# MingXiangL/SPE

Measured on AMD Instinct MI355X. Metric: images/sec (whole node) at 3x800x1333 bs=2/GPU, higher is better.
Workload: dtype bf16/fp16 operands, fp32 accumulate; 1 GPU; TSCAM_cait_S24 (C=384, depth 24, 8 heads) + 0-layer encoder + 6-layer conditional-DETR decoder x2 stages, 100 queries, COCO heads (91), 2x3x800x1333 per GPU (N=4150 tokens), fwd + SetCriterion + SetCriterionRefine + bwd + grad all-reduce + clip + AdamW; global_batch=2, parallelism=dp1

## Files before the change

### spe_amd/csrc/attn_flash_bwd.hip

```cpp
#include "attn_flash_common.h"

#define FLB_NW 4
#define FLB_HB 4
#define FLB_GWR 144
#define FLB_NK16 3
#define FLB_RSFUSE 1
#define FLB_DQAHEAD 2
#define FLB_SB_NOMEM 0x00F
#define FLB_PHASE() __builtin_amdgcn_sched_barrier(0)
#ifndef SPE_ABLATE
#undef FLB_DBG_SAMETILE
#undef FLB_DBG_NOST
#undef FLB_DBG_STAMP
#endif
#ifdef FLB_DBG_STAMP
#define FLB_STAMP(k) asm volatile("s_memtime %0\n\ts_waitcnt lgkmcnt(0)" : "=s"(stamp[k]))
#else
#define FLB_STAMP(k)
#endif
#ifndef FLB_STAGGER
#define FLB_STAGGER 1
#endif

struct FlashBwdArgs {
// ... 430 lines not shown
                for (int g = 0; g < H; ++g)
#pragma unroll
                    for (int dt = 0; dt < DT; ++dt) *reinterpret_cast<f32x4_t*>(dst + (g * DT + dt) * 256 + lane * 4) = dQ[g][dt];
            }
        }
        s += seg;
    }

#ifdef FLB_DBG_STAMP
    if (blockIdx.x == 0 && threadIdx.x == 0) {
        unsigned long long* o = reinterpret_cast<unsigned long long*>(a.dS);
        for (int k = 0; k < 5; ++k) o[k] = stacc[k];
        o[5] = stn;
    }
#endif
    {
        constexpr int NWG = 2 * (H * H + H);
        float* row = a.ws_w + ((long)blockIdx.x * NW + wave) * NWG;
        const f32x4_t dsum = (gwacc[0] + gwacc[1]) + (gwacc[2] + gwacc[3]);
        const int nn = lane & 15;
#pragma unroll
        for (int r = 0; r < 4; ++r) {
            const int g = 4 * (lane >> 4) + r;
            if (g < H && nn < H) row[g * H + nn] = FL_LN2 * dsum[r];
        }
#pragma unroll
        for (int g = 0; g < H; ++g) {
            const float v = spe_wave_sum(gb[g]);
            if (lane == 0) row[H * H + g] = v;
        }
    }
}

__global__ __launch_bounds__(256) void bwdq_dq_merge_kernel(const float* __restrict__ ws, float* __restrict__ O, unsigned short* __restrict__ O16,
                                                            long ob, long on, long oh, int B, int H, int N, int nt, int dh, int DT, int nmaj, int spw,
                                                            float scale, long nvec) {
    const long i = (long)blockIdx.x * 256 + threadIdx.x;
    if (i >= nvec) return;
    const int lane = (int)(i & 63);
    long r = i >> 6;
    const int dt = (int)(r % DT); r /= DT;
    const int g = (int)(r % H); r /= H;
    const int wave = (int)(r % FLB_NW); r /= FLB_NW;
    const long bm = r;
    const int b = (int)(bm / nmaj), mj = (int)(bm % nmaj);
    const int qt = mj * FLB_NW + wave;
    const int q = qt * 16 + (lane & 15), d = dt * 16 + 4 * (lane >> 4);
    if (qt >= nt || q >= N || d >= dh) return;
    const int first_wg = (int)((bm * nt) / spw), last_wg = (int)(((bm + 1) * nt - 1) / spw);
    const long slot_stride = (long)FLB_NW * H * DT * 256;
    const float* src = ws + bm * FL_MAXSLOT * slot_stride + ((long)wave * H + g) * (long)(DT * 256) + dt * 256 + lane * 4;
    f32x4_t acc = {0.f, 0.f, 0.f, 0.f};
    for (int sl = 0; sl <= last_wg - first_wg; ++sl) acc += *reinterpret_cast<const f32x4_t*>(src + sl * slot_stride);
    acc *= scale;
    const long oi = (long)b * ob + (long)q * on + (long)g * oh + d;
#pragma unroll
    for (int k = 0; k < 4; ++k) {
        if (d + k >= dh) break;
        if (O) O[oi + k] = acc[k];
    }
    if (O16) {
        if (d + 3 < dh && ((ob | on | oh) & 3) == 0 && ((reinterpret_cast<uintptr_t>(O16) & 7) == 0)) {
            const unsigned short h0 = spe_f2bf(acc[0]), h1 = spe_f2bf(acc[1]), h2 = spe_f2bf(acc[2]), h3 = spe_f2bf(acc[3]);
            *reinterpret_cast<uint2*>(O16 + oi) = make_uint2((unsigned)h0 | ((unsigned)h1 << 16), (unsigned)h2 | ((unsigned)h3 << 16));
        } else {
#pragma unroll
            for (int k = 0; k < 4; ++k) { if (d + k >= dh) break; O16[oi + k] = spe_f2bf(acc[k]); }
        }
    }
}

struct FlashBwdKArgs {
    const unsigned char* Qf; const unsigned char* dOf; const unsigned char* dO16;
    const unsigned char* Kf; const unsigned char* Vf;
    const float* Wl; const float* Ww; const float* bw;
    const float* c0; int Np;
    float* ws_d;
    float* ws_v;
    float* ws_w;
    const unsigned* keepbits;
    int B, N, nt, nmaj, spw; long total;
    float p_drop;
};

__device__ __forceinline__ void flb_rowsum4(const f32x4_t (&t)[4], f32x4_t& o) {
    float a0, a1, a2, a3, b0, b1, b2, b3;
    asm("s_nop 1\n\t"
        "v_add_f32_dpp %0, %12, %12 row_ror:8 row_mask:0xf bank_mask:0x3\n\t"
        "v_add_f32_dpp %1, %13, %13 row_ror:8 row_mask:0xf bank_mask:0x3\n\t"
        "v_add_f32_dpp %2, %14, %14 row_ror:8 row_mask:0xf bank_mask:0x3\n\t"
        "v_add_f32_dpp %3, %15, %15 row_ror:8 row_mask:0xf bank_mask:0x3\n\t"
        "v_add_f32_dpp %0, %20, %20 row_ror:8 row_mask:0xf bank_mask:0xc\n\t"
        "v_add_f32_dpp %1, %21, %21 row_ror:8 row_mask:0xf bank_mask:0xc\n\t"
        "v_add_f32_dpp %2, %22, %22 row_ror:8 row_mask:0xf bank_mask:0xc\n\t"
        "v_add_f32_dpp %3, %23, %23 row_ror:8 row_mask:0xf bank_mask:0xc\n\t"
        "v_add_f32_dpp %4, %16, %16 row_ror:8 row_mask:0xf bank_mask:0x3\n\t"
        "v_add_f32_dpp %5, %17, %17 row_ror:8 row_mask:0xf bank_mask:0x3\n\t"
        "v_add_f32_dpp %6, %18, %18 row_ror:8 row_mask:0xf bank_mask:0x3\n\t"
        "v_add_f32_dpp %7, %19, %19 row_ror:8 row_mask:0xf bank_mask:0x3\n\t"
        "v_add_f32_dpp %4, %24, %24 row_ror:8 row_mask:0xf bank_mask:0xc\n\t"
        "v_add_f32_dpp %5, %25, %25 row_ror:8 row_mask:0xf bank_mask:0xc\n\t"
        "v_add_f32_dpp %6, %26, %26 row_ror:8 row_mask:0xf bank_mask:0xc\n\t"
// ... 480 lines not shown
#pragma unroll
            for (int dt = 0; dt < DT; ++dt) flb_acc_fence(dV[g][dt]);
        if (wvalid) {
            float* dst = a.ws_v + (((long)bm * FL_MAXSLOT + slot) * NW + wave) * (long)(H * DT * 256);
#pragma unroll
            for (int g = 0; g < H; ++g)
#pragma unroll
                for (int dt = 0; dt < DT; ++dt) *reinterpret_cast<f32x4_t*>(dst + (g * DT + dt) * 256 + lane * 4) = dV[g][dt];
        }
        s += seg;
    }

#ifdef FLB_DBG_STAMP
    if (blockIdx.x == 0 && threadIdx.x == 0) {
        unsigned long long* o = reinterpret_cast<unsigned long long*>(a.ws_w);
        for (int k = 0; k < 6; ++k) o[k] = stacc[k];
        o[6] = stn;
    }
#endif
    {
        constexpr int NWG = 2 * (H * H + H);
        float* row = a.ws_w + ((long)blockIdx.x * NW + wave) * NWG + (H * H + H);
        const f32x4_t dsum = (gwacc[0] + gwacc[1]) + (gwacc[2] + gwacc[3]);
        const int nn = lane & 15;
#pragma unroll
        for (int r = 0; r < 4; ++r) {
            const int g = 4 * (lane >> 4) + r;
            if (g < H && nn < H) row[g * H + nn] = dsum[r] * (1.0f / FL_PD_SCALE);
            if (g < H && nn == H) row[H * H + g] = dsum[r];
        }
    }
}

__global__ __launch_bounds__(256) void bwdk_rows_merge_kernel(const float* __restrict__ ws, float* __restrict__ out, int B, int H, int N, int Np, int nmaj) {
    const long i = (long)blockIdx.x * 256 + threadIdx.x;
    const long per = (long)Np * H;
    if (i >= (long)B * per) return;
    const long bq = i / H; const int q = (int)(bq % Np), b = (int)(bq / Np);
    if (q >= N) { out[i] = 0.f; return; }
    const float* src = ws + (long)b * nmaj * per + (i - (long)b * per);
    float acc = 0.f;
    int m = 0;
    for (; m + 8 <= nmaj; m += 8) {
        float v[8];
#pragma unroll
        for (int k = 0; k < 8; ++k) v[k] = src[(long)(m + k) * per];
#pragma unroll
        for (int k = 0; k < 8; ++k) acc += v[k];
    }
    for (; m < nmaj; ++m) acc += src[(long)m * per];
    out[i] = acc;
}

constexpr int flbq_lds_bytes(int H, int DT, bool drop) {
    return (4 + FLB_NK16) * H * DT * 512 + 512 + FLB_NW * 3 * 4 * H * FLB_GWR + (drop ? 2048 : 0);
}
constexpr int flbk_lds_bytes(int H, int DT, bool drop) {
    return (4 + FLB_NK16) * H * DT * 512 + 2048 + 2 * FLB_NW * 16 * H * 4 + 512 + FLB_NW * 3 * 4 * H * FLB_GWR + (drop ? 2048 : 0);
}

static int dispatch_bwdq(const FlashBwdArgs& a, int H, int dh, int nwg, hipStream_t st) {
    return attn_dispatch(H, dh, [&](auto h, auto ds, auto tl) {
        constexpr int HH = decltype(h)::value, DS = decltype(ds)::value, DT = FragDims<DS, decltype(tl)::value>::DT;
        constexpr bool TL = decltype(tl)::value;
        if constexpr (flbq_lds_bytes(HH, DT, true) > FL_LDS_MAX) return -2;
        else return fl_launch<FlashBwdArgs, talking_bwdq_kernel<HH, DS, TL, true>, talking_bwdq_kernel<HH, DS, TL, false>>(
            a, nwg, 64 * FLB_NW, flbq_lds_bytes(HH, DT, false), flbq_lds_bytes(HH, DT, true), a.p_drop > 0.f, st);
    });
}

extern "C" int spe_talking_bwdq_plan(int B, int N, int nwg, int* steps_per_wg, int* nwg_used, int* nmajor) {
    const int nt = (N + 15) / 16;
    if ((long)B * nt <= 0 || nwg <= 0) { *steps_per_wg = 0; *nwg_used = 0; *nmajor = 0; return 0; }
    const FlashPlan p = fl_plan(B, nt, FLB_NW, nt, nwg);
    *steps_per_wg = p.spw; *nwg_used = p.nwg; *nmajor = p.nmaj;
    return 0;
}

static int bwdq_fill(FlashBwdArgs& a, FlashPlan& p, const void* Qf, const void* dOf, const void* Kf, const void* Vf, const void* K16, const float* Wl,
                     const float* Ww, const float* c0, int Np, const void* keepbits, int B, int H, int N, int dh, int nwg, float p_drop) {
    const int nt = (N + 15) / 16;
    if (dh < 1 || dh > 64 || nwg <= 0 || Np < nt * 16 || (p_drop > 0.f && !keepbits)) return -2;
    p = fl_plan(B, nt, FLB_NW, nt, nwg);
    a.Qf = (const unsigned char*)Qf; a.dOf = (const unsigned char*)dOf; a.Kf = (const unsigned char*)Kf; a.Vf = (const unsigned char*)Vf;
// ... 29 lines not shown
    return attn_dispatch(H, dh, [&](auto h, auto ds, auto tl) {
        constexpr int HH = decltype(h)::value, DS = decltype(ds)::value, DT = FragDims<DS, decltype(tl)::value>::DT;
        constexpr bool TL = decltype(tl)::value;
        if constexpr (flbk_lds_bytes(HH, DT, true) > FL_LDS_MAX) return -2;
        else return fl_launch<FlashBwdKArgs, talking_bwdk_kernel<HH, DS, TL, true>, talking_bwdk_kernel<HH, DS, TL, false>>(
            a, nwg, 64 * FLB_NW, flbk_lds_bytes(HH, DT, false), flbk_lds_bytes(HH, DT, true), a.p_drop > 0.f, st);
    });
}

extern "C" int spe_talking_fused_supported(int H, int dh) {
    return attn_dispatch(H, dh, [](auto h, auto ds, auto tl) {
        constexpr int HH = decltype(h)::value, DT = FragDims<decltype(ds)::value, decltype(tl)::value>::DT;
        return (flf_lds_bytes(HH, DT, true) <= FL_LDS_MAX && flbq_lds_bytes(HH, DT, true) <= FL_LDS_MAX && flbk_lds_bytes(HH, DT, true) <= FL_LDS_MAX) ? 0 : -2;
    }) == 0;
}

extern "C" int spe_talking_bwdk_pass1(const void* Qf, const void* dOf, const void* dO16, const void* Kf, const void* Vf, const float* Wl, const float* Ww,
                                      const float* bw, const float* c0, int Np, float* ws_d, float* ws_v, float* ws_w, float* Drows, float* dv, void* dv16,
                                      long ob, long on, long oh, const void* keepbits, int B, int H, int N, int dh, int nwg, float p_drop, hipStream_t st) {
    const int nt = (N + 15) / 16;
    if ((long)B * nt <= 0) return 0;
    if (dh < 1 || dh > 64 || nwg <= 0 || Np < nt * 16 + 64 || (p_drop > 0.f && !keepbits)) return -2;
    if (!Qf || !dOf || !dO16 || !Kf || !Vf || !Wl || !Ww || !bw || !c0 || !ws_d || !ws_v || !ws_w || !Drows || (!dv && !dv16)) return -2;
    const FlashPlan p = fl_plan(B, nt, FLB_NW, nt, nwg);
    FlashBwdKArgs a;
    a.Qf = (const unsigned char*)Qf; a.dOf = (const unsigned char*)dOf; a.dO16 = (const unsigned char*)dO16;
    a.Kf = (const unsigned char*)Kf; a.Vf = (const unsigned char*)Vf; a.Wl = Wl; a.Ww = Ww; a.bw = bw; a.c0 = c0; a.Np = Np;
    a.ws_d = ws_d; a.ws_v = ws_v; a.ws_w = ws_w;
    a.keepbits = (p_drop > 0.f) ? reinterpret_cast<const unsigned*>(keepbits) : nullptr;
    a.B = B; a.N = N; a.nt = nt; a.nmaj = p.nmaj; a.spw = p.spw; a.total = p.total; a.p_drop = p_drop;
    int rc = dispatch_bwdk(a, H, dh, p.nwg, st);
    if (rc != 0) return rc;
    const long n = (long)B * Np * H;
    hipLaunchKernelGGL(bwdk_rows_merge_kernel, dim3((unsigned)((n + 255) / 256)), dim3(256), 0, st, ws_d, Drows, B, H, N, Np, p.nmaj);
    SPE_CHECK_LAUNCH();
    const int DT = frag_geom(dh).dt;
    const long nvec = (long)B * p.nmaj * FLB_NW * H * DT * 64;
    hipLaunchKernelGGL(bwdq_dq_merge_kernel, dim3((unsigned)((nvec + 255) / 256)), dim3(256), 0, st, ws_v, dv, reinterpret_cast<unsigned short*>(dv16),
                       ob, on, oh, B, H, N, nt, dh, DT, p.nmaj, p.spw, 1.0f / FL_PD_SCALE, nvec);
    SPE_CHECK_LAUNCH();
    return 0;
}
```

### spe_amd/csrc/decoder_kv.hip

```cpp
#include <cstdlib>
#include "common.h"
#include "attn_pack.h"
#include "det_reduce.h"

typedef unsigned int kvu32x4_t __attribute__((ext_vector_type(4)));
typedef _Float16 kvh4_t __attribute__((ext_vector_type(4)));

__device__ __forceinline__ float kv_h2f(unsigned short h) { return (float)__builtin_bit_cast(_Float16, h); }

struct KvFragArgs {
    const unsigned short* ym; long ldm; const unsigned short* yp; long ldp;
    unsigned short* Kf; unsigned short* V16; unsigned short* K16; unsigned short* Vf;
    int L, B, S, H, dh, nt;
};

#define KV_MAXDH 64
__global__ __launch_bounds__(256) void kv_frag_kernel(KvFragArgs a) {
    __shared__ __attribute__((aligned(16))) unsigned short sK[4][16 * (2 * KV_MAXDH + 8)];
    __shared__ __attribute__((aligned(16))) unsigned short sV[4][16 * (KV_MAXDH + 8)];
    const int lane = threadIdx.x & 63, wave = __builtin_amdgcn_readfirstlane(threadIdx.x >> 6);
    const int dh = a.dh, dk = 2 * dh, d = a.H * dh, nt = a.nt, S = a.S;
    const int LDK = dk + 8, LDV = dh + 8;
    const int PPK = dk / 8, PPV = dh / 8, PPR = PPK + PPV;
    const int steps_k = (dk + 31) / 32, steps_v = (dh + 31) / 32, DTk = (dk + 15) / 16, DTv = (dh + 15) / 16;
// ... 96 lines not shown
extern "C" int spe_kv_grad_scatter(const float* dk, const float* dv, void* dYm, long ldm, void* dYp, long ldp, int layer, int B, int S,
                                   int H, int dh, hipStream_t st) {
    const long rows = (long)B * S;
    if (rows <= 0) return 0;
    if ((dh & 3) || (ldm & 3) || (ldp & 3) || layer < 0) return -2;
    const long n = rows * H * 3 * (dh / 4);
    long nb = (n + 255) / 256; if (nb > 8192) nb = 8192;
    hipLaunchKernelGGL(kv_grad_scatter_kernel, dim3((unsigned)nb), dim3(256), 0, st, dk, dv, reinterpret_cast<unsigned short*>(dYm), ldm,
                       reinterpret_cast<unsigned short*>(dYp), ldp, layer, rows, H, dh);
    SPE_CHECK_LAUNCH();
    return 0;
}


#define KV_MAXBLK 32
struct ColsumBlkArgs { const unsigned short* x; long ld; long R; int nblk, blkC, accumulate; float* out[KV_MAXBLK]; };
__global__ __launch_bounds__(256) void colsum_bf16_blocks_kernel(ColsumBlkArgs a, DetWs ws) {
    __shared__ float red[4][64];
    const int cl = threadIdx.x & 63, rl = threadIdx.x >> 6;
    const int C = a.nblk * a.blkC, c = blockIdx.x * 64 + cl;
    float acc = 0.f;
    if (c < C)
        for (long r = (long)blockIdx.y * 4 + rl; r < a.R; r += (long)gridDim.y * 4) acc += spe_bf2f(a.x[r * a.ld + c]);
    red[rl][cl] = acc;
    __syncthreads();
    det_reduce(ws, blockIdx.x, blockIdx.y, gridDim.y, 64, threadIdx.x, 256,
               [&](int k) { return red[0][k] + red[1][k] + red[2][k] + red[3][k]; },
               [&](int k, float s) {
                   const int cc = blockIdx.x * 64 + k;
                   if (cc < C) { float* o = a.out[cc / a.blkC] + cc % a.blkC; *o = a.accumulate ? *o + s : s; }
               });
}

__global__ __launch_bounds__(256) void colsum_bf16_blocks_v8_kernel(ColsumBlkArgs a, DetWs ws) {
    __shared__ float red[8][256 + 8];
    const int cg = threadIdx.x & 31, rl = threadIdx.x >> 5;
    const int C = a.nblk * a.blkC, c0 = blockIdx.x * 256 + cg * 8;
    float acc[8] = {0.f, 0.f, 0.f, 0.f, 0.f, 0.f, 0.f, 0.f};
    if (c0 < C) {
        const long rows_per = (a.R + gridDim.y - 1) / gridDim.y;
        const long r0 = (long)blockIdx.y * rows_per, r1 = r0 + rows_per < a.R ? r0 + rows_per : a.R;
        for (long r = r0 + rl; r < r1; r += 8) {
            const uint4 q = *reinterpret_cast<const uint4*>(a.x + r * a.ld + c0);
            const unsigned w[4] = {q.x, q.y, q.z, q.w};
#pragma unroll
            for (int i = 0; i < 4; ++i) { acc[2 * i] += __uint_as_float(w[i] << 16); acc[2 * i + 1] += __uint_as_float(w[i] & 0xffff0000u); }
        }
    }
#pragma unroll
    for (int i = 0; i < 8; ++i) red[rl][cg * 8 + i] = acc[i];
    __syncthreads();
    det_reduce(ws, blockIdx.x, blockIdx.y, gridDim.y, 256, threadIdx.x, 256,
               [&](int k) { float t = 0.f;
#pragma unroll
                            for (int j = 0; j < 8; ++j) t += red[j][k];
                            return t; },
               [&](int k, float s) {
                   const int cc = blockIdx.x * 256 + k;
                   if (cc < C) { float* o = a.out[cc / a.blkC] + cc % a.blkC; *o = a.accumulate ? *o + s : s; }
               });
}

extern "C" int spe_colsum_bf16_blocks(const void* x, long ld, long R, int nblk, int blkC, float* const* outs, int accumulate, hipStream_t st) {
    if (nblk <= 0 || blkC <= 0 || R <= 0) return 0;
    if (nblk > KV_MAXBLK) return -2;
    ColsumBlkArgs a;
    a.x = (const unsigned short*)x; a.ld = ld; a.R = R; a.nblk = nblk; a.blkC = blkC; a.accumulate = accumulate;
    for (int i = 0; i < nblk; ++i) a.out[i] = outs[i];
    if (((nblk * blkC) & 7) == 0 && (ld & 7) == 0 && (reinterpret_cast<uintptr_t>(x) & 15) == 0) {
        const int gx = (nblk * blkC + 255) / 256;
        static const int ry_max = SPE_KNOB("SPE_COLSUM_RY", 96);
        long ry = (R + 63) / 64; if (ry > ry_max) ry = ry_max; if (ry < 1) ry = 1;
        while (gx * ry > 1024 && ry > 16) ry /= 2;
        DetWs ws = spe_detws();
        DetDeferSeg sg[KV_MAXBLK];
        for (int i = 0; i < nblk; ++i) sg[i] = DetDeferSeg{outs[i], blkC};
        float* region = det_defer_try(gx, ry, 256, nblk, sg, st);
        if (region) ws.defer = region; else DET_CHECK(ws, gx, ry, 256);
        hipLaunchKernelGGL(colsum_bf16_blocks_v8_kernel, dim3(gx, (unsigned)ry), dim3(256), 0, st, a, ws);
        if (region) det_defer_commit(region, gx, ry, 256, nblk, sg, accumulate);
        SPE_CHECK_LAUNCH();
        return 0;
    }
    const int gx = (nblk * blkC + 63) / 64;
    long ry = (R + 255) / 256; if (ry > 64) ry = 64; if (ry < 1) ry = 1;
    const DetWs ws = spe_detws();
    DET_CHECK(ws, gx, ry, 64);
    hipLaunchKernelGGL(colsum_bf16_blocks_kernel, dim3(gx, (unsigned)ry), dim3(256), 0, st, a, ws);
    SPE_CHECK_LAUNCH();
    return 0;
}
```

### spe_amd/csrc/rowops.hip

```cpp
#include "common.h"
#include "det_reduce.h"

#define LN_MAXV 4

__device__ __forceinline__ void ln_store4(float4 v, float mu, float rs, float4 g, float4 b, long ro, int c, float* __restrict__ y,
                                          unsigned short* __restrict__ y16, unsigned short* __restrict__ y16lo, bool lo_f16) {
    float4 o;
    o.x = (v.x - mu) * rs * g.x + b.x; o.y = (v.y - mu) * rs * g.y + b.y;
    o.z = (v.z - mu) * rs * g.z + b.z; o.w = (v.w - mu) * rs * g.w + b.w;
    reinterpret_cast<float4*>(y + ro)[c] = o;
    if (y16) {
        const uint2 h = spe_pack_bf16x4(o);
        *reinterpret_cast<uint2*>(y16 + ro + 4 * c) = h;
        if (y16lo) {
            const float ov[4] = {o.x, o.y, o.z, o.w};
            *reinterpret_cast<uint2*>(y16lo + ro + 4 * c) = spe_second16(ov, h, lo_f16);
        }
    }
}

template <bool RES>
__global__ __launch_bounds__(256) void ln_fwd_kernel(const float* __restrict__ x, const float* __restrict__ z,
                                                     const float* __restrict__ gamma, const float* __restrict__ beta,
                                                     float* __restrict__ sum, float* __restrict__ y,
                                                     float* __restrict__ mean, float* __restrict__ rstd,
                                                     long R, int C, float eps, unsigned short* __restrict__ y16,
                                                     unsigned short* __restrict__ y16lo, bool lo_f16, float p, uint64_t seed, uint64_t offset) {
    const int lane = threadIdx.x & 63;
    const long row = (long)blockIdx.x * 4 + (threadIdx.x >> 6);
    if (row >= R) return;
    const int C4 = C >> 2;
    const float4* xr = reinterpret_cast<const float4*>(x + row * C);
    float4 v[LN_MAXV];
    float s = 0.f;
#pragma unroll
    for (int i = 0; i < LN_MAXV; ++i) {
// ... 35 lines not shown
    const int C4 = C >> 2, ldr = C + 4;
#pragma unroll
    for (int i = 0; i < MAXV; ++i) {
        const int c = lane + 64 * i;
        if (c < C4) {
#pragma unroll
            for (int k = 0; k < K; ++k) {
                float* r = red + (long)(k * NW + w) * ldr + 4 * c;
                r[0] = acc[k][i].x; r[1] = acc[k][i].y; r[2] = acc[k][i].z; r[3] = acc[k][i].w;
            }
        }
    }
    __syncthreads();
    auto set_of = [&](int c) {
        int k = 0;
#pragma unroll
        for (int j = 1; j < K; ++j) k += c >= j * C;
        return k;
    };
    det_reduce(ws, 0, blockIdx.x, gridDim.x, K * C, threadIdx.x, NW * 64,
               [&](int c) {
                   const int k = set_of(c), cc = c - k * C;
                   float t = 0.f;
#pragma unroll
                   for (int wv = 0; wv < NW; ++wv) t += red[(long)(k * NW + wv) * ldr + cc];
                   return t;
               },
               [&](int c, float t) {
                   const int k = set_of(c);
                   store(k, c - k * C, t);
               });
}

template <int NW, bool LS, int MAXV>
__global__ __launch_bounds__(NW * 64) void ln_bwd_kernel(const float* __restrict__ dy, const float* __restrict__ x,
                                                     const float* __restrict__ gamma, const float* __restrict__ mean,
                                                     const float* __restrict__ rstd, float* __restrict__ dx,
                                                     float* __restrict__ dgamma, float* __restrict__ dbeta,
                                                     long R, int C, const float* __restrict__ add, float* __restrict__ dz,
                                                     float p, uint64_t seed, uint64_t offset, DetWs ws, const float* __restrict__ dy2,
                                                     const float* __restrict__ ls_y, const float* __restrict__ ls_gamma,
                                                     unsigned short* __restrict__ ls_dy16, float* __restrict__ ls_db, float* __restrict__ ls_dg) {
    extern __shared__ float red_raw[];
    const int lane = threadIdx.x & 63, w = threadIdx.x >> 6;
    const int C4 = C >> 2;
    const float4* g4 = reinterpret_cast<const float4*>(gamma);
    float4 ag[MAXV], ab[MAXV];
    float4 lg[LS ? MAXV : 1], lb[LS ? MAXV : 1];
#pragma unroll
    for (int i = 0; i < MAXV; ++i) { ag[i] = make_float4(0, 0, 0, 0); ab[i] = make_float4(0, 0, 0, 0); }
#pragma unroll
    for (int i = 0; i < (LS ? MAXV : 1); ++i) { lg[i] = make_float4(0, 0, 0, 0); lb[i] = make_float4(0, 0, 0, 0); }
    for (long row = (long)blockIdx.x * NW + w; row < R; row += (long)gridDim.x * NW) {
        const float4* xr = reinterpret_cast<const float4*>(x + row * C);
        const float4* dr = reinterpret_cast<const float4*>(dy + row * C);
        const float4* dr2 = dy2 ? reinterpret_cast<const float4*>(dy2 + row * C) : nullptr;
        const float mu = mean[row], rs = rstd[row];
        float4 xh[MAXV], dg[MAXV];
        float s1 = 0.f, s2 = 0.f;
#pragma unroll
        for (int i = 0; i < MAXV; ++i) {
            const int c = lane + 64 * i;
            if (c < C4) {
                const float4 xv = xr[c], g = g4[c];
                float4 dv = dr[c];
                if (dr2) dv = spe_add4(dv, dr2[c]);
                xh[i].x = (xv.x - mu) * rs; xh[i].y = (xv.y - mu) * rs; xh[i].z = (xv.z - mu) * rs; xh[i].w = (xv.w - mu) * rs;
                dg[i] = spe_mul4(dv, g);
                s1 += spe_hsum(dg[i]);
                s2 += dg[i].x * xh[i].x + dg[i].y * xh[i].y + dg[i].z * xh[i].z + dg[i].w * xh[i].w;
                spe_fma4(ag[i], dv, xh[i]);
                ab[i] = spe_add4(ab[i], dv);
            }
        }
        s1 = spe_wave_sum(s1) / (float)C;
        s2 = spe_wave_sum(s2) / (float)C;
        float4* dxr = reinterpret_cast<float4*>(dx + row * C);
        const float4* ar = add ? reinterpret_cast<const float4*>(add + row * C) : nullptr;
#pragma unroll
        for (int i = 0; i < MAXV; ++i) {
            const int c = lane + 64 * i;
            if (c < C4) {
                float4 o;
                o.x = rs * (dg[i].x - s1 - xh[i].x * s2); o.y = rs * (dg[i].y - s1 - xh[i].y * s2);
                o.z = rs * (dg[i].z - s1 - xh[i].z * s2); o.w = rs * (dg[i].w - s1 - xh[i].w * s2);
                if (ar) o = spe_add4(o, ar[c]);
                dxr[c] = o;
                if constexpr (LS) {
                    spe_fma4(lg[i], o, reinterpret_cast<const float4*>(ls_y + row * C)[c]);
                    const float4 q = spe_mul4(o, reinterpret_cast<const float4*>(ls_gamma)[c]);
                    lb[i] = spe_add4(lb[i], q);
                    *reinterpret_cast<uint2*>(ls_dy16 + row * C + 4 * c) = spe_pack_bf16x4(q);
                }
                if (dz) {
                    float ks[4];
                    spe_drop_scale4(seed, offset, (uint64_t)(row * C + 4 * c), p, ks);
                    reinterpret_cast<float4*>(dz + row * C)[c] = make_float4(o.x * ks[0], o.y * ks[1], o.z * ks[2], o.w * ks[3]);
                }
            }
        }
    }
    const float4* const acc[4] = {ag, ab, lg, lb};
    wave_cols_reduce<LS ? 4 : 2, NW, MAXV>(red_raw, acc, C, ws, [&](int k, int c, float t) {
        float* d = (k == 0) ? dgamma : ((k == 1) ? dbeta : ((k == 2) ? ls_dg : ls_db));
        d[c] += t;
    });
}

template <int NV>
__global__ __launch_bounds__(256) void ln_fwd_hw_kernel(const float* __restrict__ x, const float* __restrict__ gamma,
                                                        const float* __restrict__ beta, float* __restrict__ y,
                                                        float* __restrict__ mean, float* __restrict__ rstd,
                                                        long R, float eps, unsigned short* __restrict__ y16,
                                                        unsigned short* __restrict__ y16lo, bool lo_f16) {
    constexpr int C4 = 32 * NV, C = 4 * C4;
    const int lane = threadIdx.x & 63, hl = lane & 31;
    const long stride = (long)gridDim.x * 8;
    long row0 = ((long)blockIdx.x * 4 + (threadIdx.x >> 6)) * 2 + (lane >> 5);
    const float4* g4 = reinterpret_cast<const float4*>(gamma);
    const float4* b4 = reinterpret_cast<const float4*>(beta);
    float4 gq[NV], bq[NV];
#pragma unroll
    for (int i = 0; i < NV; ++i) { gq[i] = g4[hl + 32 * i]; bq[i] = b4[hl + 32 * i]; }
// ... 54 lines not shown
}

static int ln_fwd_launch(const float* x, const float* gamma, const float* beta, float* y, float* mean,
                         float* rstd, long R, int C, float eps, void* y16, void* y16lo, bool lo_f16, hipStream_t st) {
    if (R <= 0) return 0;
    if ((C & 3) || C > 256 * LN_MAXV || (y16lo && !y16)) return -2;
    if ((C % 128) == 0 && C <= 512) {
        static constexpr decltype(&ln_fwd_hw_kernel<1>) hw[4] = {ln_fwd_hw_kernel<1>, ln_fwd_hw_kernel<2>, ln_fwd_hw_kernel<3>, ln_fwd_hw_kernel<4>};
        long nwg_ = (R + 7) / 8; if (nwg_ > 512) nwg_ = 512;
        hipLaunchKernelGGL(hw[C / 128 - 1], dim3((unsigned)nwg_), dim3(256), 0, st, x, gamma, beta, y, mean, rstd, R, eps,
                           reinterpret_cast<unsigned short*>(y16), reinterpret_cast<unsigned short*>(y16lo), lo_f16);
        SPE_CHECK_LAUNCH();
        return 0;
    }
    return ln_fwd_rows_launch<false>(x, nullptr, gamma, beta, nullptr, y, mean, rstd, R, C, eps, y16, y16lo, lo_f16, 0.f, 0, 0, st);
}
extern "C" int spe_layernorm_fwd(const float* x, const float* gamma, const float* beta, float* y, float* mean,
                                 float* rstd, long R, int C, float eps, void* y16, void* y16lo, hipStream_t st) {
    return ln_fwd_launch(x, gamma, beta, y, mean, rstd, R, C, eps, y16, y16lo, false, st);
}
extern "C" int spe_layernorm_fwd_h(const float* x, const float* gamma, const float* beta, float* y, float* mean,
                                   float* rstd, long R, int C, float eps, void* y16, void* yh16, hipStream_t st) {
    return ln_fwd_launch(x, gamma, beta, y, mean, rstd, R, C, eps, y16, yh16, true, st);
}
static int ln_bwd_launch(const float* dy, const float* x, const float* gamma, const float* mean, const float* rstd, float* dx,
                         float* dgamma, float* dbeta, long R, int C, const float* add, float* dz, float p, uint64_t seed,
                         uint64_t offset, hipStream_t st, const float* ls_y = nullptr, const float* ls_gamma = nullptr, void* ls_dy16 = nullptr,
                         float* ls_db = nullptr, float* ls_dg = nullptr, const float* dy2 = nullptr) {
    if (R <= 0) return 0;
    if ((C & 3) || C > 256 * LN_MAXV) return -2;
    const bool ls = ls_y != nullptr;
    if (ls && (!ls_gamma || !ls_dy16 || !ls_db || !ls_dg || dz || C > 512 ||
               ((reinterpret_cast<uintptr_t>(ls_y) | reinterpret_cast<uintptr_t>(ls_gamma) | reinterpret_cast<uintptr_t>(ls_dy16)) & 15))) return -2;
    constexpr int NW = 16;
    static constexpr decltype(&ln_bwd_kernel<NW, false, 2>) kernels[3] = {ln_bwd_kernel<NW, true, 2>, ln_bwd_kernel<NW, false, 2>,
                                                                          ln_bwd_kernel<NW, false, LN_MAXV>};
    static bool attr[3] = {false, false, false};
    const int variant = ls ? 0 : (C <= 512 ? 1 : 2);
    const int nk = ls ? 4 : 2;
    if (!attr[variant]) {
        hipError_t e = hipFuncSetAttribute(reinterpret_cast<const void*>(kernels[variant]), hipFuncAttributeMaxDynamicSharedMemorySize,
                                           nk * NW * ((ls ? 512 : 256 * LN_MAXV) + 4) * (int)sizeof(float));
        if (e != hipSuccess) return (int)e;
        attr[variant] = true;
    }
    long nb = (R + NW - 1) / NW; if (nb > 256) nb = 256;
    DetWs ws = spe_detws();
    const DetDeferSeg sg[4] = {{dgamma, C}, {dbeta, C}, {ls_dg, C}, {ls_db, C}};
    float* region = det_defer_try(1, nb, nk * C, nk, sg, st);
    if (region) ws.defer = region; else DET_CHECK(ws, 1, nb, nk * C);
    hipLaunchKernelGGL(kernels[variant], dim3((unsigned)nb), dim3(NW * 64), nk * NW * (C + 4) * (int)sizeof(float), st, dy, x, gamma, mean,
                       rstd, dx, dgamma, dbeta, R, C, add, dz, p, seed, offset, ws, dy2, ls_y, ls_gamma, reinterpret_cast<unsigned short*>(ls_dy16), ls_db, ls_dg);
    if (region) det_defer_commit(region, 1, nb, nk * C, nk, sg, 1);
    SPE_CHECK_LAUNCH();
    return 0;
}
extern "C" int spe_layernorm_bwd_ls(const float* dy, const float* x, const float* gamma, const float* mean, const float* rstd, float* dx,
                                    float* dgamma, float* dbeta, long R, int C, const float* add, const float* ls_y, const float* ls_gamma,
                                    void* ls_dy16, float* ls_db, float* ls_dg, hipStream_t st) {
    if (!ls_y) return -2;
    return ln_bwd_launch(dy, x, gamma, mean, rstd, dx, dgamma, dbeta, R, C, add, nullptr, 0.f, 0, 0, st, ls_y, ls_gamma, ls_dy16, ls_db, ls_dg);
}
extern "C" int spe_layernorm_bwd(const float* dy, const float* x, const float* gamma, const float* mean,
                                 const float* rstd, float* dx, float* dgamma, float* dbeta, long R, int C,
                                 const float* add, hipStream_t st) {
    return ln_bwd_launch(dy, x, gamma, mean, rstd, dx, dgamma, dbeta, R, C, add, nullptr, 0.f, 0, 0, st);
}
extern "C" int spe_layernorm_res_bwd(const float* dy, const float* dy2, const float* sum, const float* gamma, const float* mean, const float* rstd,
                                     float* ds, float* dz, float* dgamma, float* dbeta, long R, int C, float p, uint64_t seed,
                                     uint64_t offset, hipStream_t st) {
    return ln_bwd_launch(dy, sum, gamma, mean, rstd, ds, dgamma, dbeta, R, C, nullptr, (p > 0.f) ? dz : nullptr, p, seed, offset, st,
                         nullptr, nullptr, nullptr, nullptr, nullptr, dy2);
}

__global__ __launch_bounds__(256) void softmax_fwd_kernel(const float* __restrict__ S, const unsigned char* __restrict__ mask,
                                                          float* __restrict__ P, float* __restrict__ Pd,
                                                          long rows, int rows_per_batch, int Nk, long ld,
                                                          float p_drop, uint64_t seed, uint64_t offset) {
    const int lane = threadIdx.x & 63;
    const long row = (long)blockIdx.x * 4 + (threadIdx.x >> 6);
    if (row >= rows) return;
    const float* s = S + row * ld;
    const unsigned char* mk = mask ? mask + (row / rows_per_batch) * (long)Nk : nullptr;
    float m = -INFINITY, l = 0.f;
// ... 394 lines not shown
```

Baseline: 42.24 images/sec.

## Fuse bwdk merge kernels, widen colsum unrolling, prefetch rows in LayerNorm backward

```diff
diff --git a/spe_amd/csrc/attn_flash_bwd.hip b/spe_amd/csrc/attn_flash_bwd.hip
--- a/spe_amd/csrc/attn_flash_bwd.hip
+++ b/spe_amd/csrc/attn_flash_bwd.hip
@@ -486,10 +486,9 @@
     }
 }
 
-__global__ __launch_bounds__(256) void bwdq_dq_merge_kernel(const float* __restrict__ ws, float* __restrict__ O, unsigned short* __restrict__ O16,
-                                                            long ob, long on, long oh, int B, int H, int N, int nt, int dh, int DT, int nmaj, int spw,
-                                                            float scale, long nvec) {
-    const long i = (long)blockIdx.x * 256 + threadIdx.x;
+__device__ __forceinline__ void bwdq_dq_merge_body(long i, const float* __restrict__ ws, float* __restrict__ O, unsigned short* __restrict__ O16,
+                                                   long ob, long on, long oh, int B, int H, int N, int nt, int dh, int DT, int nmaj, int spw,
+                                                   float scale, long nvec) {
     if (i >= nvec) return;
     const int lane = (int)(i & 63);
     long r = i >> 6;
@@ -522,6 +521,11 @@
             for (int k = 0; k < 4; ++k) { if (d + k >= dh) break; O16[oi + k] = spe_f2bf(acc[k]); }
         }
     }
+}
+__global__ __launch_bounds__(256) void bwdq_dq_merge_kernel(const float* __restrict__ ws, float* __restrict__ O, unsigned short* __restrict__ O16,
+                                                            long ob, long on, long oh, int B, int H, int N, int nt, int dh, int DT, int nmaj, int spw,
+                                                            float scale, long nvec) {
+    bwdq_dq_merge_body((long)blockIdx.x * 256 + threadIdx.x, ws, O, O16, ob, on, oh, B, H, N, nt, dh, DT, nmaj, spw, scale, nvec);
 }
 
 struct FlashBwdKArgs {
@@ -1068,8 +1072,7 @@
     }
 }
 
-__global__ __launch_bounds__(256) void bwdk_rows_merge_kernel(const float* __restrict__ ws, float* __restrict__ out, int B, int H, int N, int Np, int nmaj) {
-    const long i = (long)blockIdx.x * 256 + threadIdx.x;
+__device__ __forceinline__ void bwdk_rows_merge_body(long i, const float* __restrict__ ws, float* __restrict__ out, int B, int H, int N, int Np, int nmaj) {
     const long per = (long)Np * H;
     if (i >= (long)B * per) return;
     const long bq = i / H; const int q = (int)(bq % Np), b = (int)(bq / Np);
@@ -1086,6 +1089,13 @@
     }
     for (; m < nmaj; ++m) acc += src[(long)m * per];
     out[i] = acc;
+}
+__global__ __launch_bounds__(256) void bwdk_merges_kernel(const float* __restrict__ ws_d, float* __restrict__ Drows, int Np, unsigned rows_blocks,
+                                                          const float* __restrict__ ws_v, float* __restrict__ dv, unsigned short* __restrict__ dv16,
+                                                          long ob, long on, long oh, int B, int H, int N, int nt, int dh, int DT, int nmaj, int spw,
+                                                          float scale, long nvec) {
+    if (blockIdx.x < rows_blocks) bwdk_rows_merge_body((long)blockIdx.x * 256 + threadIdx.x, ws_d, Drows, B, H, N, Np, nmaj);
+    else bwdq_dq_merge_body((long)(blockIdx.x - rows_blocks) * 256 + threadIdx.x, ws_v, dv, dv16, ob, on, oh, B, H, N, nt, dh, DT, nmaj, spw, scale, nvec);
 }
 
 constexpr int flbq_lds_bytes(int H, int DT, bool drop) {
@@ -1181,12 +1191,11 @@
     int rc = dispatch_bwdk(a, H, dh, p.nwg, st);
     if (rc != 0) return rc;
     const long n = (long)B * Np * H;
-    hipLaunchKernelGGL(bwdk_rows_merge_kernel, dim3((unsigned)((n + 255) / 256)), dim3(256), 0, st, ws_d, Drows, B, H, N, Np, p.nmaj);
-    SPE_CHECK_LAUNCH();
     const int DT = frag_geom(dh).dt;
     const long nvec = (long)B * p.nmaj * FLB_NW * H * DT * 64;
-    hipLaunchKernelGGL(bwdq_dq_merge_kernel, dim3((unsigned)((nvec + 255) / 256)), dim3(256), 0, st, ws_v, dv, reinterpret_cast<unsigned short*>(dv16),
-                       ob, on, oh, B, H, N, nt, dh, DT, p.nmaj, p.spw, 1.0f / FL_PD_SCALE, nvec);
+    const unsigned rows_blocks = (unsigned)((n + 255) / 256);
+    hipLaunchKernelGGL(bwdk_merges_kernel, dim3(rows_blocks + (unsigned)((nvec + 255) / 256)), dim3(256), 0, st, ws_d, Drows, Np, rows_blocks,
+                       ws_v, dv, reinterpret_cast<unsigned short*>(dv16), ob, on, oh, B, H, N, nt, dh, DT, p.nmaj, p.spw, 1.0f / FL_PD_SCALE, nvec);
     SPE_CHECK_LAUNCH();
     return 0;
 }
diff --git a/spe_amd/csrc/decoder_kv.hip b/spe_amd/csrc/decoder_kv.hip
--- a/spe_amd/csrc/decoder_kv.hip
+++ b/spe_amd/csrc/decoder_kv.hip
@@ -152,31 +152,46 @@
                });
 }
 
+template <int CG>
 __global__ __launch_bounds__(256) void colsum_bf16_blocks_v8_kernel(ColsumBlkArgs a, DetWs ws) {
-    __shared__ float red[8][256 + 8];
-    const int cg = threadIdx.x & 31, rl = threadIdx.x >> 5;
-    const int C = a.nblk * a.blkC, c0 = blockIdx.x * 256 + cg * 8;
-    float acc[8] = {0.f, 0.f, 0.f, 0.f, 0.f, 0.f, 0.f, 0.f};
+    constexpr int RL = 256 / CG, CW = CG * 8;
+    __shared__ float red[RL][CW + 8];
+    const int cg = threadIdx.x % CG, rl = threadIdx.x / CG;
+    const int C = a.nblk * a.blkC, c0 = blockIdx.x * CW + cg * 8;
+    float acc[4][8];
+#pragma unroll
+    for (int j = 0; j < 4; ++j)
+#pragma unroll
+        for (int i = 0; i < 8; ++i) acc[j][i] = 0.f;
     if (c0 < C) {
         const long rows_per = (a.R + gridDim.y - 1) / gridDim.y;
         const long r0 = (long)blockIdx.y * rows_per, r1 = r0 + rows_per < a.R ? r0 + rows_per : a.R;
-        for (long r = r0 + rl; r < r1; r += 8) {
-            const uint4 q = *reinterpret_cast<const uint4*>(a.x + r * a.ld + c0);
+        const unsigned short* src = a.x + c0;
+        auto add8 = [](float (&s)[8], const uint4& q) {
             const unsigned w[4] = {q.x, q.y, q.z, q.w};
 #pragma unroll
-            for (int i = 0; i < 4; ++i) { acc[2 * i] += __uint_as_float(w[i] << 16); acc[2 * i + 1] += __uint_as_float(w[i] & 0xffff0000u); }
-        }
-    }
-#pragma unroll
-    for (int i = 0; i < 8; ++i) red[rl][cg * 8 + i] = acc[i];
+            for (int i = 0; i < 4; ++i) { s[2 * i] += __uint_as_float(w[i] << 16); s[2 * i + 1] += __uint_as_float(w[i] & 0xffff0000u); }
+        };
+        long r = r0 + rl;
+        for (; r + 7 * RL < r1; r += 8 * RL) {
+            uint4 q[8];
+#pragma unroll
+            for (int k = 0; k < 8; ++k) q[k] = *reinterpret_cast<const uint4*>(src + (r + k * RL) * a.ld);
+#pragma unroll
+            for (int k = 0; k < 8; ++k) add8(acc[k & 3], q[k]);
+        }
+        for (; r < r1; r += RL) add8(acc[0], *reinterpret_cast<const uint4*>(src + r * a.ld));
+    }
+#pragma unroll
+    for (int i = 0; i < 8; ++i) red[rl][cg * 8 + i] = (acc[0][i] + acc[1][i]) + (acc[2][i] + acc[3][i]);
     __syncthreads();
-    det_reduce(ws, blockIdx.x, blockIdx.y, gridDim.y, 256, threadIdx.x, 256,
+    det_reduce(ws, blockIdx.x, blockIdx.y, gridDim.y, CW, threadIdx.x, 256,
                [&](int k) { float t = 0.f;
 #pragma unroll
-                            for (int j = 0; j < 8; ++j) t += red[j][k];
+                            for (int j = 0; j < RL; ++j) t += red[j][k];
                             return t; },
                [&](int k, float s) {
-                   const int cc = blockIdx.x * 256 + k;
+                   const int cc = blockIdx.x * CW + k;
                    if (cc < C) { float* o = a.out[cc / a.blkC] + cc % a.blkC; *o = a.accumulate ? *o + s : s; }
                });
 }
@@ -188,17 +203,22 @@
     a.x = (const unsigned short*)x; a.ld = ld; a.R = R; a.nblk = nblk; a.blkC = blkC; a.accumulate = accumulate;
     for (int i = 0; i < nblk; ++i) a.out[i] = outs[i];
     if (((nblk * blkC) & 7) == 0 && (ld & 7) == 0 && (reinterpret_cast<uintptr_t>(x) & 15) == 0) {
-        const int gx = (nblk * blkC + 255) / 256;
+        const int Ct = nblk * blkC, rem = Ct % 256;
+        const bool narrow = rem > 0 && rem <= 128;
+        const int CW = narrow ? 128 : 256, RL = narrow ? 16 : 8;
+        const int gx = (Ct + CW - 1) / CW;
         static const int ry_max = SPE_KNOB("SPE_COLSUM_RY", 96);
-        long ry = (R + 63) / 64; if (ry > ry_max) ry = ry_max; if (ry < 1) ry = 1;
+        long ry = (R + 8 * RL - 1) / (8 * RL);
+        if (ry > ry_max) ry = ry_max; if (ry < 1) ry = 1;
         while (gx * ry > 1024 && ry > 16) ry /= 2;
         DetWs ws = spe_detws();
         DetDeferSeg sg[KV_MAXBLK];
         for (int i = 0; i < nblk; ++i) sg[i] = DetDeferSeg{outs[i], blkC};
-        float* region = det_defer_try(gx, ry, 256, nblk, sg, st);
-        if (region) ws.defer = region; else DET_CHECK(ws, gx, ry, 256);
-        hipLaunchKernelGGL(colsum_bf16_blocks_v8_kernel, dim3(gx, (unsigned)ry), dim3(256), 0, st, a, ws);
-        if (region) det_defer_commit(region, gx, ry, 256, nblk, sg, accumulate);
+        float* region = det_defer_try(gx, ry, CW, nblk, sg, st);
+        if (region) ws.defer = region; else DET_CHECK(ws, gx, ry, CW);
+        if (narrow) hipLaunchKernelGGL(colsum_bf16_blocks_v8_kernel<16>, dim3(gx, (unsigned)ry), dim3(256), 0, st, a, ws);
+        else hipLaunchKernelGGL(colsum_bf16_blocks_v8_kernel<32>, dim3(gx, (unsigned)ry), dim3(256), 0, st, a, ws);
+        if (region) det_defer_commit(region, gx, ry, CW, nblk, sg, accumulate);
         SPE_CHECK_LAUNCH();
         return 0;
     }
diff --git a/spe_amd/csrc/rowops.hip b/spe_amd/csrc/rowops.hip
--- a/spe_amd/csrc/rowops.hip
+++ b/spe_amd/csrc/rowops.hip
@@ -2,6 +2,30 @@
 #include "det_reduce.h"
 
 #define LN_MAXV 4
+
+static long spe_balanced_blocks(long R, int per_wg, long wg_slots) {
+    static const int balanced = SPE_KNOB("SPE_LN_BALANCED", 1);
+    if (wg_slots < 1) wg_slots = 1;
+    if (!balanced) { const long nb = (R + per_wg - 1) / per_wg; return nb < wg_slots ? nb : wg_slots; }
+    const long per_round = wg_slots * per_wg;
+    const long k = (R + per_round - 1) / per_round;
+    return (R + k * per_wg - 1) / (k * per_wg);
+}
+static int spe_resident_workgroups(const void* fn, int threads, int smem) {
+    int per_cu = 0, dev = 0, cus = 0;
+    if (hipOccupancyMaxActiveBlocksPerMultiprocessor(&per_cu, fn, threads, (size_t)smem) != hipSuccess || per_cu < 1) per_cu = 1;
+    if (hipGetDevice(&dev) != hipSuccess || hipDeviceGetAttribute(&cus, hipDeviceAttributeMultiprocessorCount, dev) != hipSuccess || cus < 1) cus = 256;
+    return per_cu * cus;
+}
+#ifndef LN_BWD_NW_LS
+#define LN_BWD_NW_LS 12
+#endif
+#ifndef LN_BWD_NW
+#define LN_BWD_NW 8
+#endif
+#ifndef LN_BWD_NW_WIDE
+#define LN_BWD_NW_WIDE 12
+#endif
 
 __device__ __forceinline__ void ln_store4(float4 v, float mu, float rs, float4 g, float4 b, long ro, int c, float* __restrict__ y,
                                           unsigned short* __restrict__ y16, unsigned short* __restrict__ y16lo, bool lo_f16) {
@@ -103,6 +127,11 @@
                });
 }
 
+__device__ __forceinline__ float4 ln_add4_unfused(float4 a, float4 b) {
+#pragma clang fp contract(off)
+    return make_float4(a.x + b.x, a.y + b.y, a.z + b.z, a.w + b.w);
+}
+
 template <int NW, bool LS, int MAXV>
 __global__ __launch_bounds__(NW * 64) void ln_bwd_kernel(const float* __restrict__ dy, const float* __restrict__ x,
                                                      const float* __restrict__ gamma, const float* __restrict__ mean,
@@ -113,29 +142,74 @@
                                                      const float* __restrict__ ls_y, const float* __restrict__ ls_gamma,
                                                      unsigned short* __restrict__ ls_dy16, float* __restrict__ ls_db, float* __restrict__ ls_dg) {
     extern __shared__ float red_raw[];
-    const int lane = threadIdx.x & 63, w = threadIdx.x >> 6;
+    const int lane = threadIdx.x & 63, w = __builtin_amdgcn_readfirstlane(threadIdx.x >> 6);
     const int C4 = C >> 2;
     const float4* g4 = reinterpret_cast<const float4*>(gamma);
+    constexpr bool AHEAD = MAXV <= 2;
     float4 ag[MAXV], ab[MAXV];
     float4 lg[LS ? MAXV : 1], lb[LS ? MAXV : 1];
-#pragma unroll
-    for (int i = 0; i < MAXV; ++i) { ag[i] = make_float4(0, 0, 0, 0); ab[i] = make_float4(0, 0, 0, 0); }
-#pragma unroll
-    for (int i = 0; i < (LS ? MAXV : 1); ++i) { lg[i] = make_float4(0, 0, 0, 0); lb[i] = make_float4(0, 0, 0, 0); }
-    for (long row = (long)blockIdx.x * NW + w; row < R; row += (long)gridDim.x * NW) {
-        const float4* xr = reinterpret_cast<const float4*>(x + row * C);
-        const float4* dr = reinterpret_cast<const float4*>(dy + row * C);
-        const float4* dr2 = dy2 ? reinterpret_cast<const float4*>(dy2 + row * C) : nullptr;
-        const float mu = mean[row], rs = rstd[row];
+    float4 gq[AHEAD ? MAXV : 1], lq[LS ? MAXV : 1];
+    unsigned ql[MAXV];
+    auto ld4 = [](const float* rowp, unsigned off) { return *reinterpret_cast<const float4*>(reinterpret_cast<const char*>(rowp) + off); };
+#pragma unroll
+    for (int i = 0; i < MAXV; ++i) {
+        ag[i] = make_float4(0, 0, 0, 0); ab[i] = make_float4(0, 0, 0, 0);
+        const int c = lane + 64 * i;
+        ql[i] = 16u * (unsigned)((AHEAD && c >= C4) ? C4 - 1 : c);
+        if constexpr (AHEAD) gq[i] = ld4(gamma, ql[i]);
+    }
+#pragma unroll
+    for (int i = 0; i < (LS ? MAXV : 1); ++i) {
+        lg[i] = make_float4(0, 0, 0, 0); lb[i] = make_float4(0, 0, 0, 0);
+        if constexpr (LS) lq[i] = ld4(ls_gamma, ql[i]);
+    }
+    const long stride = (long)gridDim.x * NW;
+    long row = (long)blockIdx.x * NW + w;
+    float4 nx[MAXV], nd[MAXV], nd2[(!LS && AHEAD) ? MAXV : 1];
+    float nmu = 0.f, nrs = 0.f;
+    auto request = [&](long r) {
+#pragma unroll
+        for (int i = 0; i < MAXV; ++i) {
+            if (AHEAD || lane + 64 * i < C4) {
+                nx[i] = ld4(x + r * C, ql[i]); nd[i] = ld4(dy + r * C, ql[i]);
+                if constexpr (!AHEAD) { if (dy2) nd[i] = spe_add4(nd[i], ld4(dy2 + r * C, ql[i])); }
+            }
+        }
+        if constexpr (!LS && AHEAD) {
+            if (dy2) {
+#pragma unroll
+                for (int i = 0; i < MAXV; ++i) nd2[i] = ld4(dy2 + r * C, ql[i]);
+            }
+        }
+        nmu = mean[r]; nrs = rstd[r];
+    };
+    if constexpr (AHEAD) { if (row < R) request(row); }
+    for (; row < R; row += stride) {
+        if constexpr (!AHEAD) request(row);
+        const float mu = nmu, rs = nrs;
+        const float4* ar = add ? reinterpret_cast<const float4*>(add + row * C) : nullptr;
+        float4 av[AHEAD ? MAXV : 1], lv[LS ? MAXV : 1];
+        if constexpr (AHEAD) {
+            if (ar) {
+#pragma unroll
+                for (int i = 0; i < MAXV; ++i) av[i] = ld4(add + row * C, ql[i]);
+            }
+        }
+        if constexpr (LS) {
+#pragma unroll
+            for (int i = 0; i < MAXV; ++i) lv[i] = ld4(ls_y + row * C, ql[i]);
+        }
         float4 xh[MAXV], dg[MAXV];
         float s1 = 0.f, s2 = 0.f;
 #pragma unroll
         for (int i = 0; i < MAXV; ++i) {
             const int c = lane + 64 * i;
             if (c < C4) {
-                const float4 xv = xr[c], g = g4[c];
-                float4 dv = dr[c];
-                if (dr2) dv = spe_add4(dv, dr2[c]);
+                float4 g;
+                if constexpr (AHEAD) g = gq[i]; else g = g4[c];
+                const float4 xv = nx[i];
+                float4 dv = nd[i];
+                if constexpr (!LS && AHEAD) { if (dy2) dv = spe_add4(dv, nd2[i]); }
                 xh[i].x = (xv.x - mu) * rs; xh[i].y = (xv.y - mu) * rs; xh[i].z = (xv.z - mu) * rs; xh[i].w = (xv.w - mu) * rs;
                 dg[i] = spe_mul4(dv, g);
                 s1 += spe_hsum(dg[i]);
@@ -144,10 +218,10 @@
                 ab[i] = spe_add4(ab[i], dv);
             }
         }
+        if constexpr (AHEAD) { if (row + stride < R) request(row + stride); }
         s1 = spe_wave_sum(s1) / (float)C;
         s2 = spe_wave_sum(s2) / (float)C;
         float4* dxr = reinterpret_cast<float4*>(dx + row * C);
-        const float4* ar = add ? reinterpret_cast<const float4*>(add + row * C) : nullptr;
 #pragma unroll
         for (int i = 0; i < MAXV; ++i) {
             const int c = lane + 64 * i;
@@ -155,11 +229,13 @@
                 float4 o;
                 o.x = rs * (dg[i].x - s1 - xh[i].x * s2); o.y = rs * (dg[i].y - s1 - xh[i].y * s2);
                 o.z = rs * (dg[i].z - s1 - xh[i].z * s2); o.w = rs * (dg[i].w - s1 - xh[i].w * s2);
-                if (ar) o = spe_add4(o, ar[c]);
+                if (ar) {
+                    if constexpr (AHEAD) o = ln_add4_unfused(o, av[i]); else o = spe_add4(o, ar[c]);
+                }
                 dxr[c] = o;
                 if constexpr (LS) {
-                    spe_fma4(lg[i], o, reinterpret_cast<const float4*>(ls_y + row * C)[c]);
-                    const float4 q = spe_mul4(o, reinterpret_cast<const float4*>(ls_gamma)[c]);
+                    spe_fma4(lg[i], o, lv[i]);
+                    const float4 q = spe_mul4(o, lq[i]);
                     lb[i] = spe_add4(lb[i], q);
                     *reinterpret_cast<uint2*>(ls_dy16 + row * C + 4 * c) = spe_pack_bf16x4(q);
                 }
@@ -280,24 +356,30 @@
     const bool ls = ls_y != nullptr;
     if (ls && (!ls_gamma || !ls_dy16 || !ls_db || !ls_dg || dz || C > 512 ||
                ((reinterpret_cast<uintptr_t>(ls_y) | reinterpret_cast<uintptr_t>(ls_gamma) | reinterpret_cast<uintptr_t>(ls_dy16)) & 15))) return -2;
-    constexpr int NW = 16;
-    static constexpr decltype(&ln_bwd_kernel<NW, false, 2>) kernels[3] = {ln_bwd_kernel<NW, true, 2>, ln_bwd_kernel<NW, false, 2>,
-                                                                          ln_bwd_kernel<NW, false, LN_MAXV>};
+    static constexpr decltype(&ln_bwd_kernel<LN_BWD_NW, false, 2>) kernels[3] = {ln_bwd_kernel<LN_BWD_NW_LS, true, 2>, ln_bwd_kernel<LN_BWD_NW, false, 2>,
+                                                                                 ln_bwd_kernel<LN_BWD_NW_WIDE, false, LN_MAXV>};
+    static constexpr int nws[3] = {LN_BWD_NW_LS, LN_BWD_NW, LN_BWD_NW_WIDE};
     static bool attr[3] = {false, false, false};
+    static int slots_C[3] = {0, 0, 0}, slots[3] = {0, 0, 0};
     const int variant = ls ? 0 : (C <= 512 ? 1 : 2);
-    const int nk = ls ? 4 : 2;
+    const int nk = ls ? 4 : 2, NW = nws[variant];
+    const int smem = nk * NW * (C + 4) * (int)sizeof(float);
     if (!attr[variant]) {
         hipError_t e = hipFuncSetAttribute(reinterpret_cast<const void*>(kernels[variant]), hipFuncAttributeMaxDynamicSharedMemorySize,
                                            nk * NW * ((ls ? 512 : 256 * LN_MAXV) + 4) * (int)sizeof(float));
         if (e != hipSuccess) return (int)e;
         attr[variant] = true;
     }
-    long nb = (R + NW - 1) / NW; if (nb > 256) nb = 256;
+    if (slots_C[variant] != C) {
+        slots[variant] = spe_resident_workgroups(reinterpret_cast<const void*>(kernels[variant]), NW * 64, smem);
+        slots_C[variant] = C;
+    }
+    const long nb = spe_balanced_blocks(R, NW, slots[variant]);
     DetWs ws = spe_detws();
     const DetDeferSeg sg[4] = {{dgamma, C}, {dbeta, C}, {ls_dg, C}, {ls_db, C}};
     float* region = det_defer_try(1, nb, nk * C, nk, sg, st);
     if (region) ws.defer = region; else DET_CHECK(ws, 1, nb, nk * C);
-    hipLaunchKernelGGL(kernels[variant], dim3((unsigned)nb), dim3(NW * 64), nk * NW * (C + 4) * (int)sizeof(float), st, dy, x, gamma, mean,
+    hipLaunchKernelGGL(kernels[variant], dim3((unsigned)nb), dim3(NW * 64), smem, st, dy, x, gamma, mean,
                        rstd, dx, dgamma, dbeta, R, C, add, dz, p, seed, offset, ws, dy2, ls_y, ls_gamma, reinterpret_cast<unsigned short*>(ls_dy16), ls_db, ls_dg);
     if (region) det_defer_commit(region, 1, nb, nk * C, nk, sg, 1);
     SPE_CHECK_LAUNCH();
```

Measured after the change: 42.04 images/sec. About the same (-0.5%).
